# SamuelSchlesinger/anonymous-credit-tokens

Measured on NVIDIA B200. Metric: spend_verify_refund_per_sec, higher is better.
Workload: dtype u32 limbs (256-bit modular integer)

## Files before the change

### anonymous-credit-tokens_b200/csrc/act_device.cuh

```cuda
#pragma once
#include "blake3.cuh"
#include "fe25519.cuh"
#include "ge25519.cuh"
#include "sc25519.cuh"

#define ACT_ST_OK 0
#define ACT_ST_INVALID_ISSUANCE_REQUEST_PROOF 1
#define ACT_ST_INVALID_ISSUANCE_RESPONSE_PROOF 2
#define ACT_ST_INVALID_REFUND_PROOF 4
#define ACT_ST_IDENTITY_POINT 6
#define ACT_ST_INVALID_CLIENT_SPEND_PROOF 7
#define ACT_ST_DECODE_INVALID_POINT 0x81

#define ACT_FLAG_BAD_POINT 1u
#define ACT_FLAG_IDENTITY 2u
#define ACT_FLAG_BAD_PROOF 4u

#define ACT_L 128
#define ACT_PROOF_WORDS (526 * 8)
#define ACT_ITEMS 390
#define ACT_ITEM_WORDS (ACT_ITEMS * 8)
#define ACT_SPEND_BYTES 15784u
#define ACT_SPEND_CHUNKS 16

#ifndef ACT_FB_BITS
#define ACT_FB_BITS 13
#endif
#ifndef ACT_FB_BITS_HOT
#define ACT_FB_BITS_HOT 16
#endif
#define ACT_FB_PART 512
#define ACT_FB_BATCH 16
#if defined(__CUDACC__)
#define ACT_HD __host__ __device__ __forceinline__
#else
#define ACT_HD static inline
#endif
struct fb_tab {
    const ge_niels* p;
    u32 bits, win, ent;
};
ACT_HD u32 fb_win_of(u32 bits) { return (253u + bits) / bits; }
ACT_HD u32 fb_ent_of(u32 bits) { return (1u << (bits - 1)) + 1u; }
ACT_HD size_t fb_size_of(u32 bits) { return (size_t)fb_win_of(bits) * fb_ent_of(bits); }
ACT_HD u32 fb_parts_of(u32 bits) { u32 n = fb_ent_of(bits) - 1; return n >= ACT_FB_PART ? n / ACT_FB_PART : 1; }
#define ACT_CT_WIN 64
#define ACT_CT_ENT 9
#define ACT_CT_SIZE (ACT_CT_WIN * ACT_CT_ENT)

#ifndef ACT_RANGE_SPLIT
#define ACT_RANGE_SPLIT 4
#endif

#define ACT_BASE_G 0
#define ACT_BASE_H1 1
#define ACT_BASE_H2 2
#define ACT_BASE_H3 3
#define ACT_BASE_W 4
#define ACT_FB_BASES 5

struct act_ctx {
    fb_tab fb[ACT_FB_BASES];
    const ge_niels* ct_g;
    sc x;
    ge W;
    ge W_half;
    u32 h_enc[3][8];
    u32 prefix[4][48];
    u32 prefix_len[4];
};
#define ACT_TR_REQUEST 0
#define ACT_TR_RESPOND 1
#define ACT_TR_REFUND 2
#define ACT_TR_SPEND 3

#if ACT_PTX
#define ACT_ATOMIC_OR(p, v) atomicOr((p), (v))
#else
#define ACT_ATOMIC_OR(p, v) (*(p) |= (v))
#endif

ACT_FN void load8(u32* w, const u32* p) {
#if ACT_PTX
    uint4 a = __ldg(reinterpret_cast<const uint4*>(p));
    uint4 b = __ldg(reinterpret_cast<const uint4*>(p) + 1);
    w[0] = a.x; w[1] = a.y; w[2] = a.z; w[3] = a.w; w[4] = b.x; w[5] = b.y; w[6] = b.z; w[7] = b.w;
#else
    for (int i = 0; i < 8; i++) w[i] = p[i];
#endif
}
ACT_FN void store8(u32* p, const u32* w) {
#if ACT_PTX
    reinterpret_cast<uint4*>(p)[0] = make_uint4(w[0], w[1], w[2], w[3]);
    reinterpret_cast<uint4*>(p)[1] = make_uint4(w[4], w[5], w[6], w[7]);
#else
    for (int i = 0; i < 8; i++) p[i] = w[i];
#endif
}
ACT_FN void load8_rw(u32* w, const u32* p) {
#if ACT_PTX
    uint4 a = reinterpret_cast<const uint4*>(p)[0];
    uint4 b = reinterpret_cast<const uint4*>(p)[1];
    w[0] = a.x; w[1] = a.y; w[2] = a.z; w[3] = a.w; w[4] = b.x; w[5] = b.y; w[6] = b.z; w[7] = b.w;
#else
    for (int i = 0; i < 8; i++) w[i] = p[i];
#endif
}
ACT_FN void store8_zero(u32* p) {
    u32 z[8] = {0, 0, 0, 0, 0, 0, 0, 0};
    store8(p, z);
}
ACT_FN sc load_scalar(const u32* p) { u32 w[8]; load8(w, p); return sc_from_words(w); }
// ... 141 lines not shown
        if (k < M - 1) {
            ACT_NOUNROLL for (int d = 0; d < 4 * WIN; d++) Q = ge_dbl_u<VT>(Q, d == 4 * WIN - 1);
        }
    }
}
template <int M>
ACT_FN ge vb_mul_split_neg(const vb_table* t, const sc& s) {
    const int WIN = 64 / M;
    sc b = sc_bias<4>(s);
    ge a = ge_identity();
    ACT_NOUNROLL for (int i = WIN - 1; i >= 0; i--) {
        if (i != WIN - 1) {
            ACT_NOUNROLL for (int d = 0; d < 4; d++) {
#if ACT_PREFETCH >= 2
                if (d == 3) {
                    int d0 = sc_digit<4>(b, i);
                    prefetch_line(&t[0].e[d0 < 0 ? -d0 : d0]);
                }
#endif
                a = ge_dbl_u<true>(a, d == 3);
            }
        }
        ACT_NOUNROLL for (int k = 0; k < M; k++) {
            if (k + 1 < M) {
                int dn = sc_digit<4>(b, (k + 1) * WIN + i);
                prefetch_line(&t[k + 1].e[dn < 0 ? -dn : dn]);
            }
            int dk = sc_digit<4>(b, k * WIN + i);
            a = ge_add_cached_u<true>(a, tab_load(&t[k], (u32)(dk < 0 ? -dk : dk)), dk < 0 ? 0u : 1u, k + 1 < M || i == 0);
        }
    }
    return a;
}
#ifndef ACT_RANGE_BUCKETS
#define ACT_RANGE_BUCKETS 1
#endif
#if ACT_RANGE_BUCKETS
ACT_FN u32* bucket_ptr(vb_table* t, u32 idx) { return reinterpret_cast<u32*>(&t[idx / 9].e[idx % 9]); }
ACT_FN void bucket_store(vb_table* t, u32 idx, const ge& p) {
    u32* q = bucket_ptr(t, idx);
    store8(q, p.X.v); store8(q + 8, p.Y.v); store8(q + 16, p.Z.v); store8(q + 24, p.T.v);
}
ACT_FN ge bucket_load(vb_table* t, u32 idx) {
    ge p;
    const u32* q = bucket_ptr(t, idx);
    load8_rw(p.X.v, q); load8_rw(p.Y.v, q + 8); load8_rw(p.Z.v, q + 16); load8_rw(p.T.v, q + 24);
    return p;
}
#ifndef ACT_BUCKET_SKIP0
#define ACT_BUCKET_SKIP0 0
#endif
ACT_FN void vb_pair_buckets_fill(const ge& P, const sc& s0, const sc& s1, vb_table* t) {
    sc b0 = sc_bias<4>(s0), b1 = sc_bias<4>(s1);
    {
        ge id = ge_identity();
        ACT_NOUNROLL for (u32 k = 0; k < 18; k++) bucket_store(t, k, id);
    }
    ge Q = P;
    ACT_NOUNROLL for (int i = 0; i < 64; i++) {
        ge_cached Qc = ge_to_cached(Q);
        ACT_NOUNROLL for (int r = 0; r < 2; r++) {
            int d = sc_digit<4>(r ? b1 : b0, i);
#if ACT_BUCKET_SKIP0
            u32 ad = (u32)(d < 0 ? -d : d);
            u32 idx = 9u * (u32)r + (ad ? ad : 1u);
            if (i + 1 < 64 || r == 0) {
                int dn = r ? sc_digit<4>(b0, i + 1) : sc_digit<4>(b1, i);
                u32 an = (u32)(dn < 0 ? -dn : dn);
                prefetch_line(bucket_ptr(t, 9u * (u32)(r ^ 1) + (an ? an : 1u)));
            }
            ge B = bucket_load(t, idx);
            B = ge_add_cached_u<true>(B, Qc, d < 0 ? 0u : 1u, true);
            if (ad) bucket_store(t, idx, B);
#else
            u32 idx = 9u * (u32)r + (u32)(d < 0 ? -d : d);
            if (i + 1 < 64 || r == 0) {
                int dn = r ? sc_digit<4>(b0, i + 1) : sc_digit<4>(b1, i);
                prefetch_line(bucket_ptr(t, 9u * (u32)(r ^ 1) + (u32)(dn < 0 ? -dn : dn)));
            }
            ge B = bucket_load(t, idx);
            B = ge_add_cached_u<true>(B, Qc, d < 0 ? 0u : 1u, true);
            bucket_store(t, idx, B);
#endif
        }
        if (i + 1 < 64) {
            ACT_NOUNROLL for (int k = 0; k < 4; k++) Q = ge_dbl_u<true>(Q, k == 3);
        }
    }
}
ACT_FN ge vb_pair_buckets_sum(vb_table* t, int r) {
    ge S = bucket_load(t, 9u * (u32)r + 8u), R = S;
    ACT_NOUNROLL for (u32 d = 7; d >= 1; d--) {
        S = ge_add_cached_u<true>(S, ge_to_cached(bucket_load(t, 9u * (u32)r + d)), 0u, true);
        R = ge_add_cached_u<true>(R, ge_to_cached(S), 0u, true);
    }
    return R;
}
#endif

ACT_NOINLINE void vb_mul_ct_(ge* out, const ge* P, const sc* s) {
    vb_table t;
    vb_table_build(&t, *P);
    sc b = sc_bias<4>(*s);
    ge acc = ge_identity();
    ACT_NOUNROLL for (int i = 63; i >= 0; i--) {
        if (i != 63) {
            acc = ge_dbl(acc, false); acc = ge_dbl(acc, false); acc = ge_dbl(acc, false); acc = ge_dbl(acc, true);
        }
        acc = ge_add_cached(acc, vb_lookup_ct(&t, sc_digit<4>(b, i)));
    }
    *out = acc;
}

#ifndef ACT_SIGN_SPLIT
#define ACT_SIGN_SPLIT 4
#endif
ACT_NOINLINE void vb_mul2_ct_(ge* out1, ge* out2, const ge* P, const sc* s1, const sc* s2) {
    const int M = ACT_SIGN_SPLIT, WIN = 64 / M;
    vb_table t[M];
    vb_split_tables<M>(*P, t);
    ACT_NOUNROLL for (int w = 0; w < 2; w++) {
        sc b = sc_bias<4>(w ? *s2 : *s1);
        ge a = ge_identity();
        ACT_NOUNROLL for (int i = WIN - 1; i >= 0; i--) {
            if (i != WIN - 1) {
                ACT_NOUNROLL for (int d = 0; d < 4; d++) a = ge_dbl_u(a, d == 3);
            }
            ACT_NOUNROLL for (int k = 0; k < M; k++) a = ge_add_cached_u(a, vb_lookup_ct(&t[k], sc_digit<4>(b, k * WIN + i)), 0u, k + 1 < M || i == 0);
        }
        if (w) *out2 = a; else *out1 = a;
// ... 154 lines not shown
    vb_table_build(&t[1], *X_A);
    sc ss[2] = {*z, *gamma};
    bool ng[2] = {false, true};
    ge Y_A = vb_mul_multi<2>(t, ss, ng);
    ge Y_G = fb_accumulate(ge_identity(), C->fb[ACT_BASE_G], sc_sub(*z, sc_mul(*e, *gamma)), false);
    Y_G = fb_accumulate(Y_G, C->fb[ACT_BASE_W], *gamma, true);
    tr_small tr;
    u32 w[8];
    tr_init(&tr, C, kind);
    if (kind == ACT_TR_RESPOND) tr_add32(&tr, c->v);
    tr_add32(&tr, e->v);
    tr_add32(&tr, A_words);
    ristretto_encode_(w, X_A); tr_add32(&tr, w);
    ristretto_encode_(w, &X_G); tr_add32(&tr, w);
    ristretto_encode_(w, &Y_A); tr_add32(&tr, w);
    ristretto_encode_(w, &Y_G); tr_add32(&tr, w);
    sc g2 = tr_challenge(&tr);
    return sc_eq(g2, *gamma);
}
ACT_FN void issuance_check_thread(const act_ctx* C, size_t i, const u32* Kin, const u32* resp, u8* status) {
    const u32* rs = resp + 40 * i;
    ge K, A;
    u32 aw[8];
    load8(aw, rs);
    u32 valid = load_point(&K, Kin + 8 * i) & ristretto_decode_(&A, aw);
    sc e = load_scalar(rs + 8), gamma = load_scalar(rs + 16), z = load_scalar(rs + 24), c = load_scalar(rs + 32);
    ge X_A = ge_add(K, ge_basepoint());
    X_A = fb_accumulate(X_A, C->fb[ACT_BASE_H1], c, false);
    u32 ok = dleq_check_(C, ACT_TR_RESPOND, &c, &e, &gamma, &z, aw, &A, &X_A);
    status[i] = (u8)(!valid ? ACT_ST_DECODE_INVALID_POINT : (ok ? ACT_ST_OK : ACT_ST_INVALID_ISSUANCE_RESPONSE_PROOF));
}

ACT_FN void spend_range_thread(const act_ctx* C, size_t p, int j, const u32* proofs, u32* items, u32* com_niels, u32* flags,
                               vb_table* tabs , u32* cpts ) {
    const u32* pf = proofs + (size_t)ACT_PROOF_WORDS * p;
    u32* it = items + (size_t)ACT_ITEM_WORDS * p;
    u32 cw[8];
    load8(cw, pf + 8 * (4 + j));
    ge P;
    u32 valid = ristretto_decode_(&P, cw);
    if (!valid) ACT_ATOMIC_OR(&flags[p], ACT_FLAG_BAD_POINT);
    store8(it + 8 * (5 + j), cw);
    {
        ge_niels n = ge_affine_to_niels(P.X, P.Y);
        u32* cn = com_niels + ((size_t)ACT_L * p + j) * 24;
        store_fe(cn, n.ypx); store_fe(cn + 8, n.ymx); store_fe(cn + 16, n.xy2d);
    }
#if ACT_RANGE_BUCKETS
    {
        sc g0 = load_scalar(pf + 8 * (140 + j));
        sc g1 = sc_sub(load_scalar(pf + 8 * 132), g0);
        vb_pair_buckets_fill(P, sc_half(g0), sc_half(g1), tabs);
    }
#else
    vb_split_tables<ACT_RANGE_SPLIT, true>(P, tabs);
#endif
    u32* cp = cpts + ((size_t)2 * ACT_L * p + 2 * j) * 32;
    ACT_NOUNROLL for (int b = 0; b < 2; b++) {
#if ACT_RANGE_BUCKETS
        ge Q = vb_pair_buckets_sum(tabs, b);
#else
        sc gb = load_scalar(pf + 8 * (140 + j));
        if (b) gb = sc_sub(load_scalar(pf + 8 * 132), gb);
        gb = sc_half(gb);
        ge Q = vb_mul_split_neg<ACT_RANGE_SPLIT>(tabs, gb);
#endif
        ACT_NOUNROLL for (int t = 0; t < 2; t++) {
            int tab;
            sc s;
            if (t == 0) { tab = ACT_BASE_H3; s = load_scalar(pf + 8 * (268 + 2 * j + b)); }
            else { if (!b) continue; tab = ACT_BASE_H1; s = sc_sub(load_scalar(pf + 8 * 132), load_scalar(pf + 8 * (140 + j))); }
            Q = fb_accumulate(Q, C->fb[tab], sc_half(s), false);
        }
        store_fe(cp + 32 * b, Q.X); store_fe(cp + 32 * b + 8, Q.Y); store_fe(cp + 32 * b + 16, Q.Z); store_fe(cp + 32 * b + 24, Q.T);
    }
}

#ifndef ACT_ENC_BATCH
#define ACT_ENC_BATCH 64
#endif
ACT_FN void spend_encode_thread(const act_ctx* C, size_t p, int part, const u32* cpts, u32* items, int pts = 2 * ACT_L, int item0 = 133) {
    (void)C;
    const u32* src = cpts + ((size_t)pts * p + (size_t)part * ACT_ENC_BATCH) * 32;
    u32* dst = items + (size_t)ACT_ITEM_WORDS * p + 8 * (item0 + part * ACT_ENC_BATCH);
    fe prefix[ACT_ENC_BATCH];
    fe acc = fe_one();
    ACT_NOUNROLL for (int i = 0; i < ACT_ENC_BATCH; i++) {
        ge P;
        load_fe(&P.X, src + 32 * i); load_fe(&P.Y, src + 32 * i + 8); load_fe(&P.Z, src + 32 * i + 16); load_fe(&P.T, src + 32 * i + 24);
        ge_dbl_enc s = ge_dbl_enc_prepare(P);
        fe t = fe_mul(s.eg, s.fh);
        t = fe_select(t, fe_one(), fe_is_zero(t));
        prefix[i] = acc;
        acc = fe_mul(acc, t);
    }
    fe inv = fe_invert(acc);
    ACT_NOUNROLL for (int i = ACT_ENC_BATCH - 1; i >= 0; i--) {
        ge P;
        load_fe(&P.X, src + 32 * i); load_fe(&P.Y, src + 32 * i + 8); load_fe(&P.Z, src + 32 * i + 16); load_fe(&P.T, src + 32 * i + 24);
        ge_dbl_enc s = ge_dbl_enc_prepare(P);
        fe t = fe_mul(s.eg, s.fh);
        u32 zero = fe_is_zero(t);
        t = fe_select(t, fe_one(), zero);
        fe inv_i = fe_mul(inv, prefix[i]);
        inv = fe_mul(inv, t);
        u32 w[8];
        ge_dbl_enc_finish(w, s, inv_i);
        ACT_UNROLL for (int k = 0; k < 8; k++) w[k] = zero ? 0u : w[k];
// ... 233 lines not shown
```

### anonymous-credit-tokens_b200/csrc/act_engine.cu

```cuda
#include <cuda_runtime.h>
#include <stdio.h>
#include <stdlib.h>
#include <string.h>
#include <sys/random.h>

#include <mutex>
#include <string>
#include <thread>
#include <vector>

#include "../../include/act_engine.h"
#include "act_device.cuh"
#include "act_aux.cuh"
#include "act_prove.cuh"
#include "act_store.cuh"

#ifndef ACT_ISSUE_BLOCK
#define ACT_ISSUE_BLOCK 128
#endif
#ifndef ACT_HEAD_BLOCK
#define ACT_HEAD_BLOCK 64
#endif
#ifndef ACT_SIGN_BLOCK
#define ACT_SIGN_BLOCK 64
// ... 15 lines not shown
__global__ void __launch_bounds__(ACT_SIGN_BLOCK, ACT_SIGN_BPS) refund_sign_seq_kernel(const act_ctx* C, size_t n, const u32* proofs, const u32* rnd, const u32* kprime, const u8* status,
                                                                           u32* refunds, u32* nullifiers, const u32* rnd_index, const u32* kwords) {
    size_t p = (size_t)blockIdx.x * blockDim.x + threadIdx.x;
    if (p < n) refund_sign_thread(C, p, proofs, rnd, kprime, status, refunds, nullifiers, rnd_index, kwords);
}
__global__ void __launch_bounds__(ACT_ISSUE_BLOCK, ACT_ISSUE_BPS) issuance_check_kernel(const act_ctx* C, size_t n, const u32* K, const u32* resp, u8* status) {
    size_t i = (size_t)blockIdx.x * blockDim.x + threadIdx.x;
    if (i < n) issuance_check_thread(C, i, K, resp, status);
}
#ifndef ACT_RANGE_BLOCKS_PER_SM
#define ACT_RANGE_BLOCKS_PER_SM 4
#endif
#ifndef ACT_RANGE_DYNAMIC
#define ACT_RANGE_DYNAMIC 1
#endif
#ifndef ACT_RANGE_BLOCK
#define ACT_RANGE_BLOCK 128
#endif
#if !ACT_RANGE_DYNAMIC && ACT_RANGE_BLOCK != ACT_L
#error "the static work distribution needs one block per proof"
#endif
#define ACT_RANGE_UNITS (ACT_L / 32)
#if ACT_RANGE_TRACE
__device__ unsigned long long act_trace_buf[4096 * 4];
__device__ __forceinline__ unsigned long long act_gtime() { unsigned long long t; asm volatile("mov.u64 %0, %%globaltimer;" : "=l"(t)); return t; }
#endif
#ifdef ACT_RANGE_MAXREG
#define ACT_RANGE_BOUNDS __maxnreg__(ACT_RANGE_MAXREG)
#else
#define ACT_RANGE_BOUNDS __launch_bounds__(ACT_RANGE_BLOCK, ACT_RANGE_BLOCKS_PER_SM)
#endif
__global__ void ACT_RANGE_BOUNDS spend_range_kernel(const act_ctx* C, size_t m, const u32* proofs, u32* items, u32* com_niels, u32* flags, vb_table* tabs, u32* cpts, u32* counter) {
    vb_table* mine = tabs + ((size_t)blockIdx.x * ACT_RANGE_BLOCK + threadIdx.x) * ACT_RANGE_SPLIT;
#if ACT_RANGE_TRACE
    unsigned long long t0 = act_gtime(), units = 0;
#endif
#if ACT_RANGE_DYNAMIC
    const u32 lane = threadIdx.x & 31u, total = (u32)m * ACT_RANGE_UNITS;
    for (;;) {
        u32 unit = 0;
        if (lane == 0) unit = atomicAdd(counter, 1u);
        unit = __shfl_sync(0xffffffffu, unit, 0);
        if (unit >= total) break;
        spend_range_thread(C, unit / ACT_RANGE_UNITS, (int)((unit % ACT_RANGE_UNITS) * 32 + lane), proofs, items, com_niels, flags, mine, cpts);
#if ACT_RANGE_TRACE
        units++;
#endif
    }
#else
    (void)counter;
    for (size_t p = blockIdx.x; p < m; p += gridDim.x) {
        spend_range_thread(C, p, threadIdx.x, proofs, items, com_niels, flags, mine, cpts);
#if ACT_RANGE_TRACE
        units++;
#endif
    }
#endif
#if ACT_RANGE_TRACE
    if ((threadIdx.x & 31) == 0) {
        unsigned smid; asm volatile("mov.u32 %0, %%smid;" : "=r"(smid));
        unsigned w = blockIdx.x * (ACT_RANGE_BLOCK / 32) + threadIdx.x / 32;
        if (w < 4096) { act_trace_buf[4 * w] = smid; act_trace_buf[4 * w + 1] = t0; act_trace_buf[4 * w + 2] = act_gtime(); act_trace_buf[4 * w + 3] = units; }
    }
#endif
}
#if ACT_RANGE_TRACE
extern "C" __attribute__((visibility("default"))) int act_debug_read_trace(unsigned long long* out, size_t n) {
    return (int)cudaMemcpyFromSymbol(out, act_trace_buf, n * sizeof(unsigned long long));
}
#endif
#define ACT_ENC_BLOCK 128
#define ACT_ENC_PARTS (2 * ACT_L / ACT_ENC_BATCH)
__global__ void __launch_bounds__(ACT_ENC_BLOCK, 4) spend_encode_kernel(const act_ctx* C, size_t m, const u32* cpts, u32* items, int pts, int item0) {
    size_t t = (size_t)blockIdx.x * blockDim.x + threadIdx.x;
    int parts = pts / ACT_ENC_BATCH;
    if (t < m * parts) spend_encode_thread(C, t / parts, (int)(t % parts), cpts, items, pts, item0);
}
__global__ void __launch_bounds__(ACT_L, 4) prove_range_kernel(const act_ctx* C, prove_rng R, size_t m, const u32* tokens, const u32* charges, u32* cpts) {
    for (size_t p = blockIdx.x; p < m; p += gridDim.x) prove_range_thread(C, &R, p, p, threadIdx.x, tokens, charges, cpts);
}
__global__ void __launch_bounds__(ACT_HEAD_BLOCK, ACT_HEAD_BPS) prove_head_kernel(const act_ctx* C, prove_rng R, size_t m, const u32* tokens, u32* items, u32* aux, u8* status) {
    size_t p = (size_t)blockIdx.x * blockDim.x + threadIdx.x;
    if (p < m) prove_head_thread(C, &R, p, p, tokens, items, aux, status);
}
__global__ void __launch_bounds__(ACT_HASH_BLOCK) prove_challenge_kernel(size_t m, const u32* cvs, u32* gammas) {
// ... 1556 lines not shown
```

### anonymous-credit-tokens_b200/csrc/fe25519.cuh

```cuda
#pragma once
#include <stdint.h>

#if defined(__CUDACC__)
#define ACT_FN __device__ __forceinline__
#define ACT_NOINLINE __device__ __noinline__
#define ACT_CONST __device__ __constant__ const
#else
#define ACT_FN static inline
#define ACT_NOINLINE static
#define ACT_CONST static const
#endif

#if defined(__CUDA_ARCH__)
#define ACT_PTX 1
#define ACT_UNROLL _Pragma("unroll")
#define ACT_NOUNROLL _Pragma("unroll 1")
#else
#define ACT_PTX 0
#define ACT_UNROLL
#define ACT_NOUNROLL
#endif

#ifndef ACT_REDUCE_ALT
#define ACT_REDUCE_ALT 1
// ... 548 lines not shown
        "madc.lo.cc.u32 %14, %23, %23, %14;\n\t"
        "madc.hi.u32 %15, %23, %23, %15;"
        : "+r"(r[0]), "+r"(r[1]), "+r"(r[2]), "+r"(r[3]), "+r"(r[4]), "+r"(r[5]), "+r"(r[6]), "+r"(r[7]), "+r"(r[8]), "+r"(r[9]), "+r"(r[10]), "+r"(r[11]), "+r"(r[12]), "+r"(r[13]), "+r"(r[14]), "+r"(r[15])
        : "r"(a.v[0]), "r"(a.v[1]), "r"(a.v[2]), "r"(a.v[3]), "r"(a.v[4]), "r"(a.v[5]), "r"(a.v[6]), "r"(a.v[7]));
}

#endif

ACT_FN fe fe_sq_inl(const fe& a) {
#if ACT_PTX
    u32 r[16];
    fe_sq_wide(r, a);
    return fe_reduce512(r);
#else
    return fe_mul_inl(a, a);
#endif
}
#ifndef ACT_FE_CALLS
#define ACT_FE_CALLS 1
#endif
#if ACT_FE_CALLS
ACT_NOINLINE fe fe_mul(fe a, fe b) { return fe_mul_inl(a, b); }
ACT_NOINLINE fe fe_sq(fe a) { return fe_sq_inl(a); }
#else
ACT_FN fe fe_mul(const fe& a, const fe& b) { return fe_mul_inl(a, b); }
ACT_FN fe fe_sq(const fe& a) { return fe_sq_inl(a); }
#endif

ACT_FN fe fe_sqn(fe a, int n) {
    ACT_NOUNROLL for (int i = 0; i < n; i++) a = fe_sq(a);
    return a;
}

ACT_FN fe fe_canon(const fe& a) {
    fe r = a;
    u32 top = r.v[7] >> 31;
    r.v[7] &= 0x7fffffffu;
    u64 c = (u64)top * 19u;
    ACT_UNROLL for (int i = 0; i < 8; i++) { c += r.v[i]; r.v[i] = (u32)c; c >>= 32; }
    fe t;
    c = 19;
    ACT_UNROLL for (int i = 0; i < 8; i++) { c += r.v[i]; t.v[i] = (u32)c; c >>= 32; }
    u32 ge = t.v[7] >> 31;
    t.v[7] &= 0x7fffffffu;
    u32 m = 0u - ge;
    ACT_UNROLL for (int i = 0; i < 8; i++) r.v[i] = (r.v[i] & ~m) | (t.v[i] & m);
    return r;
}
ACT_FN u32 fe_is_negative(const fe& a) { return fe_canon(a).v[0] & 1u; }
ACT_FN u32 fe_is_zero(const fe& a) {
    fe c = fe_canon(a);
    u32 o = 0;
    ACT_UNROLL for (int i = 0; i < 8; i++) o |= c.v[i];
    return o == 0;
}
ACT_FN u32 fe_eq(const fe& a, const fe& b) { return fe_is_zero(fe_sub(a, b)); }
ACT_FN fe fe_select(const fe& x, const fe& y, u32 b) {
    fe r;
    u32 m = 0u - (b & 1u);
    ACT_UNROLL for (int i = 0; i < 8; i++) r.v[i] = (x.v[i] & ~m) | (y.v[i] & m);
    return r;
}
ACT_FN fe fe_cneg(const fe& x, u32 b) { return fe_select(x, fe_neg(x), b); }
ACT_FN fe fe_abs(const fe& x) { return fe_cneg(x, fe_is_negative(x)); }

ACT_FN fe fe_from_words(const u32* w) {
// ... 58 lines not shown
```

### anonymous-credit-tokens_b200/csrc/ge25519.cuh

```cuda
#pragma once
#include "fe25519.cuh"
#include "sc25519.cuh"

struct ge { fe X, Y, Z, T; };
struct ge_cached { fe YpX, YmX, Z, T2d; };
struct ge_niels { fe ypx, ymx, xy2d; };

ACT_FN ge ge_identity() { ge r; r.X = fe_zero(); r.Y = fe_one(); r.Z = fe_one(); r.T = fe_zero(); return r; }
ACT_FN ge ge_basepoint() { ge r; r.X = fe_const(FE_BX_); r.Y = fe_const(FE_BY_); r.Z = fe_one(); r.T = fe_const(FE_BT_); return r; }
ACT_FN ge_cached ge_cached_identity() { ge_cached r; r.YpX = fe_one(); r.YmX = fe_one(); r.Z = fe_one(); r.T2d = fe_zero(); return r; }
ACT_FN ge_niels ge_niels_identity() { ge_niels r; r.ypx = fe_one(); r.ymx = fe_one(); r.xy2d = fe_zero(); return r; }

ACT_FN ge_cached ge_to_cached(const ge& p) {
    ge_cached r;
    r.YpX = fe_add(p.Y, p.X); r.YmX = fe_sub(p.Y, p.X); r.Z = p.Z; r.T2d = fe_mul(p.T, FE_D2);
    return r;
}
ACT_FN ge ge_neg(const ge& p) { ge r; r.X = fe_neg(p.X); r.Y = p.Y; r.Z = p.Z; r.T = fe_neg(p.T); return r; }

#ifndef ACT_ALU_COPY
#define ACT_ALU_COPY 0
#endif
#if defined(__CUDACC__) && ACT_ALU_COPY
__device__ u32 act_zero_word = 0;
#endif
#if ACT_PTX && ACT_ALU_COPY
ACT_FN u32 act_zero() { return __ldg(&act_zero_word); }
ACT_FN fe fe_cp(const fe& a, u32 z) {
    fe r;
    ACT_UNROLL for (int i = 0; i < 8; i++) asm("xor.b32 %0, %1, %2;" : "=r"(r.v[i]) : "r"(a.v[i]), "r"(z));
    return r;
}
ACT_FN fe fe_mul_c(const fe& a, const fe& b, u32 z) {
    fe r = (ACT_ALU_COPY & 1) ? fe_mul(fe_cp(a, z), fe_cp(b, z)) : fe_mul(a, b);
    return (ACT_ALU_COPY & 2) ? fe_cp(r, z) : r;
}
ACT_FN fe fe_sq_c(const fe& a, u32 z) {
    fe r = (ACT_ALU_COPY & 1) ? fe_sq(fe_cp(a, z)) : fe_sq(a);
    return (ACT_ALU_COPY & 2) ? fe_cp(r, z) : r;
}
#else
ACT_FN u32 act_zero() { return 0; }
ACT_FN fe fe_mul_c(const fe& a, const fe& b, u32) { return fe_mul(a, b); }
ACT_FN fe fe_sq_c(const fe& a, u32) { return fe_sq(a); }
#endif

#ifndef ACT_GE_CALLS
#define ACT_GE_CALLS 0
#endif
#if ACT_GE_CALLS
#define ACT_GE_FN ACT_NOINLINE
// ... 57 lines not shown
    fe G0 = fe_add_x<VT>(ZZ2, TT), F0 = fe_sub_x<VT>(ZZ2, TT);
    fe G = fe_select(G0, F0, neg), F = fe_select(F0, G0, neg);
    ge r;
    r.X = GE_MUL(E, F); r.Y = GE_MUL(H, G); r.Z = GE_MUL(G, F); r.T = GE_MUL(E, H);
    return r;
}
ACT_FN ge ge_add(const ge& p, const ge& q) { return ge_add_cached(p, ge_to_cached(q)); }
ACT_FN ge ge_sub(const ge& p, const ge& q) { return ge_add_cached(p, ge_to_cached(ge_neg(q))); }

ACT_GE_FN ge ge_dbl_t(ge p) {
    u32 zc_ = act_zero(); (void)zc_;
    fe XX = GE_SQ(p.X), YY = GE_SQ(p.Y), ZZ = GE_SQ(p.Z);
    fe ZZ2 = fe_dbl_tt(ZZ);
    fe XpY2 = GE_SQ(fe_add(p.X, p.Y));
    fe Yc = fe_add_tt(YY, XX), Zc = fe_sub(YY, XX);
    fe Xc = fe_sub(XpY2, Yc), Tc = fe_sub(ZZ2, Zc);
    ge r;
    r.X = GE_MUL(Xc, Tc); r.Y = GE_MUL(Yc, Zc); r.Z = GE_MUL(Zc, Tc); r.T = GE_MUL(Xc, Yc);
    return r;
}
ACT_GE_FN ge ge_dbl_not(ge p) {
    u32 zc_ = act_zero(); (void)zc_;
    fe XX = GE_SQ(p.X), YY = GE_SQ(p.Y), ZZ = GE_SQ(p.Z);
    fe ZZ2 = fe_dbl_tt(ZZ);
    fe XpY2 = GE_SQ(fe_add(p.X, p.Y));
    fe Yc = fe_add_tt(YY, XX), Zc = fe_sub(YY, XX);
    fe Xc = fe_sub(XpY2, Yc), Tc = fe_sub(ZZ2, Zc);
    ge r;
    r.X = GE_MUL(Xc, Tc); r.Y = GE_MUL(Yc, Zc); r.Z = GE_MUL(Zc, Tc); r.T = p.T;
    return r;
}
ACT_FN ge ge_dbl(const ge& p, bool want_t) { return want_t ? ge_dbl_t(p) : ge_dbl_not(p); }

template <bool VT = false>
ACT_FN ge ge_dbl_u(const ge& p, bool want_t) {
    u32 zc_ = act_zero(); (void)zc_;
    fe XX = GE_SQ(p.X), YY = GE_SQ(p.Y);
    fe Yc = fe_add_tt(YY, XX), Zc = fe_sub_x<VT>(YY, XX);
    fe ZZ = GE_SQ(p.Z);
    fe ZZ2 = fe_dbl_tt(ZZ);
    fe Tc = fe_sub_x<VT>(ZZ2, Zc);
    fe XpY2 = GE_SQ(fe_add_x<VT>(p.X, p.Y));
    fe Xc = fe_sub_x<VT>(XpY2, Yc);
    ge r;
    r.Y = GE_MUL(Yc, Zc); r.Z = GE_MUL(Tc, Zc); r.X = GE_MUL(Tc, Xc);
    r.T = p.T;
    if (want_t) r.T = GE_MUL(Xc, Yc);
    return r;
}

ACT_FN ge_cached ge_cached_cneg(const ge_cached& q, u32 neg) {
    ge_cached r;
    r.YpX = fe_select(q.YpX, q.YmX, neg); r.YmX = fe_select(q.YmX, q.YpX, neg);
    r.Z = q.Z; r.T2d = fe_select(q.T2d, fe_neg(q.T2d), neg);
    return r;
}
ACT_FN ge_niels ge_niels_cneg(const ge_niels& q, u32 neg) {
    ge_niels r;
    r.ypx = fe_select(q.ypx, q.ymx, neg); r.ymx = fe_select(q.ymx, q.ypx, neg);
    r.xy2d = fe_select(q.xy2d, fe_neg(q.xy2d), neg);
    return r;
}
ACT_FN ge_niels ge_affine_to_niels(const fe& x, const fe& y) {
    ge_niels r;
    r.ypx = fe_add(y, x); r.ymx = fe_sub(y, x); r.xy2d = fe_mul(fe_mul(x, y), FE_D2);
    return r;
}
ACT_FN ge_niels ge_to_niels(const ge& p) {
    fe zi = fe_invert(p.Z);
    return ge_affine_to_niels(fe_mul(p.X, zi), fe_mul(p.Y, zi));
}
ACT_FN ge ge_from_niels(const ge_niels& n) {
    ge r;
    r.Y = fe_add(n.ypx, n.ymx); r.X = fe_sub(n.ypx, n.ymx); r.Z = fe_add(fe_one(), fe_one());
    fe zi = fe_invert(r.Z);
    fe x = fe_mul(r.X, zi), y = fe_mul(r.Y, zi);
    r.X = x; r.Y = y; r.Z = fe_one(); r.T = fe_mul(x, y);
    return r;
// ... 93 lines not shown
```

Before: 205,900.

## Share proof-wide wNAF scalar across warp in range bucket multiplication

Each range thread previously ran bucket-method multiplications for two per-thread scalars, g0 and (total − g0), with 18 buckets. Now one lane per warp computes a width-5 wNAF of the shared total scalar into shared memory. Every thread accumulates its own g0 buckets plus sparse wNAF buckets along one doubling chain, and the second output is derived as total·P − g0·P from the first sum. This cuts per-thread point additions, since wNAF digits are sparse, but it adds warp syncs, divergent loop control (doubling every bit with branches) and a serial wNAF computation on lane 0.

```diff
diff --git a/anonymous-credit-tokens_b200/csrc/act_device.cuh b/anonymous-credit-tokens_b200/csrc/act_device.cuh
--- a/anonymous-credit-tokens_b200/csrc/act_device.cuh
+++ b/anonymous-credit-tokens_b200/csrc/act_device.cuh
@@ -76,8 +76,10 @@
 
 #if ACT_PTX
 #define ACT_ATOMIC_OR(p, v) atomicOr((p), (v))
+#define ACT_SYNCWARP() __syncwarp()
 #else
 #define ACT_ATOMIC_OR(p, v) (*(p) |= (v))
+#define ACT_SYNCWARP() ((void)0)
 #endif
 
 ACT_FN void load8(u32* w, const u32* p) {
@@ -288,6 +290,7 @@
 #ifndef ACT_RANGE_BUCKETS
 #define ACT_RANGE_BUCKETS 1
 #endif
+#define ACT_NAF_LEN 256
 #if ACT_RANGE_BUCKETS
 ACT_FN u32* bucket_ptr(vb_table* t, u32 idx) { return reinterpret_cast<u32*>(&t[idx / 9].e[idx % 9]); }
 ACT_FN void bucket_store(vb_table* t, u32 idx, const ge& p) {
@@ -300,54 +303,68 @@
     load8_rw(p.X.v, q); load8_rw(p.Y.v, q + 8); load8_rw(p.Z.v, q + 16); load8_rw(p.T.v, q + 24);
     return p;
 }
-#ifndef ACT_BUCKET_SKIP0
-#define ACT_BUCKET_SKIP0 0
-#endif
-ACT_FN void vb_pair_buckets_fill(const ge& P, const sc& s0, const sc& s1, vb_table* t) {
-    sc b0 = sc_bias<4>(s0), b1 = sc_bias<4>(s1);
+#define ACT_NAF_W 5
+#define ACT_NAF_BUCKETS (1 << (ACT_NAF_W - 2))
+ACT_FN void sc_wnaf(signed char* naf, const sc& s) {
+    u32 carry = 0;
+    int i = 0;
+    ACT_NOUNROLL while (i < 253) {
+        u32 w = (u32)i >> 5, sh = (u32)i & 31u;
+        if (((s.v[w] >> sh) & 1u) == carry) { naf[i++] = 0; continue; }
+        u32 hi = (w + 1 < 8) ? s.v[w + 1] : 0u;
+        u32 raw = (sh ? ((s.v[w] >> sh) | (hi << (32u - sh))) : s.v[w]) & ((1u << ACT_NAF_W) - 1u);
+        int v = (int)(raw + carry);
+        carry = v > (1 << (ACT_NAF_W - 1)) ? 1u : 0u;
+        naf[i] = (signed char)(v - (int)(carry << ACT_NAF_W));
+        ACT_NOUNROLL for (int m = 1; m < ACT_NAF_W && i + m < 253; m++) naf[i + m] = 0;
+        i += ACT_NAF_W;
+    }
+}
+ACT_FN void vb_pair_buckets_fill(const ge& P, const sc& s0, const signed char* naf, vb_table* t) {
+    sc b0 = sc_bias<4>(s0);
     {
         ge id = ge_identity();
-        ACT_NOUNROLL for (u32 k = 0; k < 18; k++) bucket_store(t, k, id);
+        ACT_NOUNROLL for (u32 k = 0; k < 9 + ACT_NAF_BUCKETS; k++) bucket_store(t, k, id);
     }
     ge Q = P;
-    ACT_NOUNROLL for (int i = 0; i < 64; i++) {
+    ACT_NOUNROLL for (int k = 0; k < 253; k++) {
+        const bool r0 = (k & 3) == 0;
+        const int n = naf[k];
+        const int d = r0 ? sc_digit<4>(b0, k >> 2) : 0;
+        if (r0) prefetch_line(bucket_ptr(t, (u32)(d < 0 ? -d : d)));
+        if (n) prefetch_line(bucket_ptr(t, 9u + (u32)((n < 0 ? -n : n) >> 1)));
+        if (k) Q = ge_dbl_u<true>(Q, r0 || n);
+        if (!r0 && !n) continue;
         ge_cached Qc = ge_to_cached(Q);
-        ACT_NOUNROLL for (int r = 0; r < 2; r++) {
-            int d = sc_digit<4>(r ? b1 : b0, i);
-#if ACT_BUCKET_SKIP0
-            u32 ad = (u32)(d < 0 ? -d : d);
-            u32 idx = 9u * (u32)r + (ad ? ad : 1u);
-            if (i + 1 < 64 || r == 0) {
-                int dn = r ? sc_digit<4>(b0, i + 1) : sc_digit<4>(b1, i);
-                u32 an = (u32)(dn < 0 ? -dn : dn);
-                prefetch_line(bucket_ptr(t, 9u * (u32)(r ^ 1) + (an ? an : 1u)));
-            }
+        ACT_NOUNROLL for (int r = r0 ? 0 : 1; r < (n ? 2 : 1); r++) {
+            u32 idx, neg;
+            if (r == 0) { idx = (u32)(d < 0 ? -d : d); neg = d < 0 ? 0u : 1u; }
+            else { idx = 9u + (u32)((n < 0 ? -n : n) >> 1); neg = n < 0 ? 1u : 0u; }
             ge B = bucket_load(t, idx);
-            B = ge_add_cached_u<true>(B, Qc, d < 0 ? 0u : 1u, true);
-            if (ad) bucket_store(t, idx, B);
-#else
-            u32 idx = 9u * (u32)r + (u32)(d < 0 ? -d : d);
-            if (i + 1 < 64 || r == 0) {
-                int dn = r ? sc_digit<4>(b0, i + 1) : sc_digit<4>(b1, i);
-                prefetch_line(bucket_ptr(t, 9u * (u32)(r ^ 1) + (u32)(dn < 0 ? -dn : dn)));
-            }
-            ge B = bucket_load(t, idx);
-            B = ge_add_cached_u<true>(B, Qc, d < 0 ? 0u : 1u, true);
+            B = ge_add_cached_u<true>(B, Qc, neg, true);
             bucket_store(t, idx, B);
-#endif
-        }
-        if (i + 1 < 64) {
-            ACT_NOUNROLL for (int k = 0; k < 4; k++) Q = ge_dbl_u<true>(Q, k == 3);
-        }
-    }
-}
-ACT_FN ge vb_pair_buckets_sum(vb_table* t, int r) {
-    ge S = bucket_load(t, 9u * (u32)r + 8u), R = S;
+        }
+    }
+}
+ACT_FN ge vb_pair_buckets_sum(vb_table* t) {
+    ge S = bucket_load(t, 8u), R = S;
     ACT_NOUNROLL for (u32 d = 7; d >= 1; d--) {
-        S = ge_add_cached_u<true>(S, ge_to_cached(bucket_load(t, 9u * (u32)r + d)), 0u, true);
+        S = ge_add_cached_u<true>(S, ge_to_cached(bucket_load(t, d)), 0u, true);
         R = ge_add_cached_u<true>(R, ge_to_cached(S), 0u, true);
     }
     return R;
+}
+ACT_FN ge vb_pair_shared_second(vb_table* t, const ge& R0) {
+    ge S = bucket_load(t, 9u + ACT_NAF_BUCKETS - 1), R = S;
+    ACT_NOUNROLL for (u32 e = ACT_NAF_BUCKETS - 2; e >= 1; e--) {
+        S = ge_add_cached_u<true>(S, ge_to_cached(bucket_load(t, 9u + e)), 0u, true);
+        R = ge_add_cached_u<true>(R, ge_to_cached(S), 0u, true);
+    }
+    S = ge_add_cached_u<true>(S, ge_to_cached(bucket_load(t, 9u)), 0u, true);
+    S = ge_add_cached_u<true>(S, ge_to_cached(R0), 0u, true);
+    R = ge_dbl_u<true>(R, true);
+    R = ge_add_cached_u<true>(R, ge_to_cached(S), 0u, true);
+    return ge_neg(R);
 }
 #endif
 
@@ -569,7 +586,8 @@
 }
 
 ACT_FN void spend_range_thread(const act_ctx* C, size_t p, int j, const u32* proofs, u32* items, u32* com_niels, u32* flags,
-                               vb_table* tabs , u32* cpts ) {
+                               vb_table* tabs , u32* cpts ,
+                               signed char* naf, bool naf_writer) {
     const u32* pf = proofs + (size_t)ACT_PROOF_WORDS * p;
     u32* it = items + (size_t)ACT_ITEM_WORDS * p;
     u32 cw[8];
@@ -584,18 +602,24 @@
         store_fe(cn, n.ypx); store_fe(cn + 8, n.ymx); store_fe(cn + 16, n.xy2d);
     }
 #if ACT_RANGE_BUCKETS
-    {
-        sc g0 = load_scalar(pf + 8 * (140 + j));
-        sc g1 = sc_sub(load_scalar(pf + 8 * 132), g0);
-        vb_pair_buckets_fill(P, sc_half(g0), sc_half(g1), tabs);
-    }
+    ACT_SYNCWARP();
+    if (naf_writer) sc_wnaf(naf, sc_half(load_scalar(pf + 8 * 132)));
+    ACT_SYNCWARP();
+    vb_pair_buckets_fill(P, sc_half(load_scalar(pf + 8 * (140 + j))), naf, tabs);
 #else
+    (void)naf; (void)naf_writer;
     vb_split_tables<ACT_RANGE_SPLIT, true>(P, tabs);
 #endif
     u32* cp = cpts + ((size_t)2 * ACT_L * p + 2 * j) * 32;
     ACT_NOUNROLL for (int b = 0; b < 2; b++) {
 #if ACT_RANGE_BUCKETS
-        ge Q = vb_pair_buckets_sum(tabs, b);
+        ge Q;
+        if (b == 0) {
+            Q = vb_pair_buckets_sum(tabs);
+            bucket_store(tabs, 0, Q);
+        } else {
+            Q = vb_pair_shared_second(tabs, bucket_load(tabs, 0));
+        }
 #else
         sc gb = load_scalar(pf + 8 * (140 + j));
         if (b) gb = sc_sub(load_scalar(pf + 8 * 132), gb);
@@ -611,6 +635,11 @@
         }
         store_fe(cp + 32 * b, Q.X); store_fe(cp + 32 * b + 8, Q.Y); store_fe(cp + 32 * b + 16, Q.Z); store_fe(cp + 32 * b + 24, Q.T);
     }
+}
+ACT_FN void spend_range_thread(const act_ctx* C, size_t p, int j, const u32* proofs, u32* items, u32* com_niels, u32* flags,
+                               vb_table* tabs, u32* cpts) {
+    signed char naf[ACT_NAF_LEN];
+    spend_range_thread(C, p, j, proofs, items, com_niels, flags, tabs, cpts, naf, true);
 }
 
 #ifndef ACT_ENC_BATCH
diff --git a/anonymous-credit-tokens_b200/csrc/act_engine.cu b/anonymous-credit-tokens_b200/csrc/act_engine.cu
--- a/anonymous-credit-tokens_b200/csrc/act_engine.cu
+++ b/anonymous-credit-tokens_b200/csrc/act_engine.cu
@@ -71,6 +71,9 @@
 #endif
 __global__ void ACT_RANGE_BOUNDS spend_range_kernel(const act_ctx* C, size_t m, const u32* proofs, u32* items, u32* com_niels, u32* flags, vb_table* tabs, u32* cpts, u32* counter) {
     vb_table* mine = tabs + ((size_t)blockIdx.x * ACT_RANGE_BLOCK + threadIdx.x) * ACT_RANGE_SPLIT;
+    __shared__ signed char naf[ACT_RANGE_BLOCK / 32][ACT_NAF_LEN];
+    signed char* my_naf = naf[threadIdx.x >> 5];
+    const bool naf_writer = (threadIdx.x & 31u) == 0;
 #if ACT_RANGE_TRACE
     unsigned long long t0 = act_gtime(), units = 0;
 #endif
@@ -81,7 +84,7 @@
         if (lane == 0) unit = atomicAdd(counter, 1u);
         unit = __shfl_sync(0xffffffffu, unit, 0);
         if (unit >= total) break;
-        spend_range_thread(C, unit / ACT_RANGE_UNITS, (int)((unit % ACT_RANGE_UNITS) * 32 + lane), proofs, items, com_niels, flags, mine, cpts);
+        spend_range_thread(C, unit / ACT_RANGE_UNITS, (int)((unit % ACT_RANGE_UNITS) * 32 + lane), proofs, items, com_niels, flags, mine, cpts, my_naf, naf_writer);
 #if ACT_RANGE_TRACE
         units++;
 #endif
@@ -89,7 +92,7 @@
 #else
     (void)counter;
     for (size_t p = blockIdx.x; p < m; p += gridDim.x) {
-        spend_range_thread(C, p, threadIdx.x, proofs, items, com_niels, flags, mine, cpts);
+        spend_range_thread(C, p, threadIdx.x, proofs, items, com_niels, flags, mine, cpts, my_naf, naf_writer);
 #if ACT_RANGE_TRACE
         units++;
 #endif
```

Measured after the change: 206,800, median of 6. Within noise of the previous version (+0.5%).

## Share range-proof challenge scalar via NAF buckets instead of per-bit subtraction

Applied to the files above, without the earlier changes.

Range-proof commitment scalar multiplication now uses the bit challenge g0 and the shared challenge c separately, instead of g0 and c−g0. The second multiple is rebuilt as c·P − g0·P, with c·P accumulated through a sparse width-5 NAF digit stream during the same doubling chain. The goal is fewer bucket additions than a dense signed-4-bit second scalar. The cost is more complex control flow, extra bucket storage for the NAF digits, and a final combination step in the bucket sum.

```diff
diff --git a/anonymous-credit-tokens_b200/csrc/act_device.cuh b/anonymous-credit-tokens_b200/csrc/act_device.cuh
--- a/anonymous-credit-tokens_b200/csrc/act_device.cuh
+++ b/anonymous-credit-tokens_b200/csrc/act_device.cuh
@@ -349,6 +349,96 @@
     }
     return R;
 }
+
+#ifndef ACT_RANGE_SHARED_CHALLENGE
+#define ACT_RANGE_SHARED_CHALLENGE 1
+#endif
+#if ACT_RANGE_SHARED_CHALLENGE
+#if ACT_BUCKET_SKIP0
+#error "ACT_BUCKET_SKIP0 applies to the two-scalar bucket form only (ACT_RANGE_SHARED_CHALLENGE=0)"
+#endif
+#define ACT_NAF_NONE 256
+ACT_FN void naf5_next(const u32* s, int* k, int* d, u32* carry) {
+    int i = *k;
+    for (;;) {
+        if (i >= 256) { *k = ACT_NAF_NONE; return; }
+        u32 w = (s[i >> 5] ^ (0u - *carry)) >> (i & 31);
+        if (w) {
+#if ACT_PTX
+            i += __ffs((int)w) - 1;
+#else
+            i += __builtin_ctz(w);
+#endif
+            break;
+        }
+        i = (i | 31) + 1;
+    }
+    u32 lo = s[i >> 5] >> (i & 31);
+    if ((i & 31) > 27 && i < 224) lo |= s[(i >> 5) + 1] << (32 - (i & 31));
+    int win = (int)(lo & 31u) + (int)*carry;
+    *carry = (win & 16) ? 1u : 0u;
+    *d = win - (int)(*carry << 5);
+    *k = i;
+}
+ACT_FN void vb_pair_shared_fill(const ge& P, const sc& s0, const sc& sg, vb_table* t) {
+    {
+        ge id = ge_identity();
+        ACT_NOUNROLL for (u32 k = 0; k < 18; k++) if (k != 9) bucket_store(t, k, id);
+    }
+    sc b0 = sc_bias<4>(s0);
+    u32* sgw = bucket_ptr(t, 9);
+    store8(sgw, sg.v);
+    int nk = 0, nd = 0;
+    u32 carry = 0;
+    naf5_next(sgw, &nk, &nd, &carry);
+    {
+        int d = sc_digit<4>(b0, 0);
+        prefetch_line(bucket_ptr(t, (u32)(d < 0 ? -d : d)));
+    }
+    ge Q = P;
+    int k = 0;
+    ACT_NOUNROLL for (;;) {
+        bool win = (k & 3) == 0, naf = k == nk;
+        ge_cached Qc = ge_to_cached(Q);
+        ACT_NOUNROLL for (int r = 0; r < 2; r++) {
+            if (r ? !naf : !win) continue;
+            int d = r ? nd : sc_digit<4>(b0, k >> 2);
+            u32 ad = (u32)(d < 0 ? -d : d);
+            u32 idx = r ? 9u + ((ad + 1) >> 1) : ad;
+            if (!r && k < 252) {
+                int dn = sc_digit<4>(b0, (k >> 2) + 1);
+                prefetch_line(bucket_ptr(t, (u32)(dn < 0 ? -dn : dn)));
+            }
+            ge B = bucket_load(t, idx);
+            B = ge_add_cached_u<true>(B, Qc, d < 0 ? 0u : 1u, true);
+            bucket_store(t, idx, B);
+        }
+        if (naf) {
+            nk += 5;
+            naf5_next(sgw, &nk, &nd, &carry);
+            if (nk != ACT_NAF_NONE) prefetch_line(bucket_ptr(t, 9u + (((u32)(nd < 0 ? -nd : nd) + 1) >> 1)));
+        }
+        int e = (k | 3) + 1;
+        if (nk < e) e = nk;
+        if (e > 253) break;
+        ACT_NOUNROLL for (; k < e; k++) Q = ge_dbl_u<true>(Q, k + 1 == e);
+    }
+}
+ACT_FN ge vb_pair_shared_sum(vb_table* t, int r) {
+    ge S = bucket_load(t, 9u * (u32)r + 8u), R = S;
+    ACT_NOUNROLL for (u32 d = 7; d >= 1; d--) {
+        S = ge_add_cached_u<true>(S, ge_to_cached(bucket_load(t, 9u * (u32)r + d)), 0u, true);
+        R = ge_add_cached_u<true>(R, ge_to_cached(S), 0u, true);
+    }
+    if (r == 0) {
+        bucket_store(t, 9, R);
+        return R;
+    }
+    R = ge_dbl_u<true>(R, true);
+    R = ge_add_cached_u<true>(R, ge_to_cached(S), 1u, true);
+    return ge_add_cached_u<true>(R, ge_to_cached(bucket_load(t, 9)), 1u, true);
+}
+#endif
 #endif
 
 ACT_NOINLINE void vb_mul_ct_(ge* out, const ge* P, const sc* s) {
@@ -583,7 +673,9 @@
         u32* cn = com_niels + ((size_t)ACT_L * p + j) * 24;
         store_fe(cn, n.ypx); store_fe(cn + 8, n.ymx); store_fe(cn + 16, n.xy2d);
     }
-#if ACT_RANGE_BUCKETS
+#if ACT_RANGE_BUCKETS && ACT_RANGE_SHARED_CHALLENGE
+    vb_pair_shared_fill(P, sc_half(load_scalar(pf + 8 * (140 + j))), sc_half(load_scalar(pf + 8 * 132)), tabs);
+#elif ACT_RANGE_BUCKETS
     {
         sc g0 = load_scalar(pf + 8 * (140 + j));
         sc g1 = sc_sub(load_scalar(pf + 8 * 132), g0);
@@ -594,7 +686,9 @@
 #endif
     u32* cp = cpts + ((size_t)2 * ACT_L * p + 2 * j) * 32;
     ACT_NOUNROLL for (int b = 0; b < 2; b++) {
-#if ACT_RANGE_BUCKETS
+#if ACT_RANGE_BUCKETS && ACT_RANGE_SHARED_CHALLENGE
+        ge Q = vb_pair_shared_sum(tabs, b);
+#elif ACT_RANGE_BUCKETS
         ge Q = vb_pair_buckets_sum(tabs, b);
 #else
         sc gb = load_scalar(pf + 8 * (140 + j));
```

Measured after the change: 205,800 before, 209,700 after, median of 6. +1.9%, better.

## Precompute cached chain points and use small-constant cached conversion in bucket MSM

Applied to the files above, without the earlier changes.

The bucket fill now computes all 64 doubled chain points first and stores them in cached form in the thread's scratch, instead of interleaving doubling with the bucket adds. The cached conversion replaces the full field multiply by 2d with small-constant multiplies on a scaled, negated representation (the lambda trick), and the sign flags are flipped to match. The doubling in the precompute uses inlined field ops, and the range split grows to 10 tables so the scratch can hold the 64 extra points. This trades a larger per-thread local-memory footprint and more stores and loads for fewer full multiplies and a better-separated dependency chain.

```diff
diff --git a/anonymous-credit-tokens_b200/csrc/act_device.cuh b/anonymous-credit-tokens_b200/csrc/act_device.cuh
--- a/anonymous-credit-tokens_b200/csrc/act_device.cuh
+++ b/anonymous-credit-tokens_b200/csrc/act_device.cuh
@@ -48,8 +48,11 @@
 #define ACT_CT_ENT 9
 #define ACT_CT_SIZE (ACT_CT_WIN * ACT_CT_ENT)
 
+#ifndef ACT_RANGE_BUCKETS
+#define ACT_RANGE_BUCKETS 1
+#endif
 #ifndef ACT_RANGE_SPLIT
-#define ACT_RANGE_SPLIT 4
+#define ACT_RANGE_SPLIT (ACT_RANGE_BUCKETS ? 10 : 4)
 #endif
 
 #define ACT_BASE_G 0
@@ -285,10 +288,8 @@
     }
     return a;
 }
-#ifndef ACT_RANGE_BUCKETS
-#define ACT_RANGE_BUCKETS 1
-#endif
 #if ACT_RANGE_BUCKETS
+static_assert(ACT_RANGE_SPLIT * 9 >= 18 + 64, "the bucket form keeps 18 buckets and 64 chain points in the thread's scratch");
 ACT_FN u32* bucket_ptr(vb_table* t, u32 idx) { return reinterpret_cast<u32*>(&t[idx / 9].e[idx % 9]); }
 ACT_FN void bucket_store(vb_table* t, u32 idx, const ge& p) {
     u32* q = bucket_ptr(t, idx);
@@ -300,52 +301,51 @@
     load8_rw(p.X.v, q); load8_rw(p.Y.v, q + 8); load8_rw(p.Z.v, q + 16); load8_rw(p.T.v, q + 24);
     return p;
 }
-#ifndef ACT_BUCKET_SKIP0
-#define ACT_BUCKET_SKIP0 0
-#endif
+ACT_FN void cached_store(vb_table* t, u32 idx, const ge_cached& c) {
+    u32* q = bucket_ptr(t, idx);
+    store8(q, c.YpX.v); store8(q + 8, c.YmX.v); store8(q + 16, c.Z.v); store8(q + 24, c.T2d.v);
+}
+ACT_FN ge_cached cached_load(vb_table* t, u32 idx) {
+    ge_cached c;
+    const u32* q = bucket_ptr(t, idx);
+    load8_rw(c.YpX.v, q); load8_rw(c.YmX.v, q + 8); load8_rw(c.Z.v, q + 16); load8_rw(c.T2d.v, q + 24);
+    return c;
+}
 ACT_FN void vb_pair_buckets_fill(const ge& P, const sc& s0, const sc& s1, vb_table* t) {
+    {
+        ge Q = P;
+        ACT_NOUNROLL for (u32 i = 0;; i++) {
+            cached_store(t, 18u + i, ge_to_cached_neg_pub(Q));
+            if (i == 63) break;
+            ACT_NOUNROLL for (int k = 0; k < 4; k++) Q = ge_dbl_u<true, true>(Q, k == 3);
+        }
+    }
     sc b0 = sc_bias<4>(s0), b1 = sc_bias<4>(s1);
     {
         ge id = ge_identity();
         ACT_NOUNROLL for (u32 k = 0; k < 18; k++) bucket_store(t, k, id);
     }
-    ge Q = P;
     ACT_NOUNROLL for (int i = 0; i < 64; i++) {
-        ge_cached Qc = ge_to_cached(Q);
+        ge_cached Qc = cached_load(t, 18u + (u32)i);
+        if (i + 1 < 64) prefetch_line(bucket_ptr(t, 19u + (u32)i));
         ACT_NOUNROLL for (int r = 0; r < 2; r++) {
             int d = sc_digit<4>(r ? b1 : b0, i);
-#if ACT_BUCKET_SKIP0
-            u32 ad = (u32)(d < 0 ? -d : d);
-            u32 idx = 9u * (u32)r + (ad ? ad : 1u);
-            if (i + 1 < 64 || r == 0) {
-                int dn = r ? sc_digit<4>(b0, i + 1) : sc_digit<4>(b1, i);
-                u32 an = (u32)(dn < 0 ? -dn : dn);
-                prefetch_line(bucket_ptr(t, 9u * (u32)(r ^ 1) + (an ? an : 1u)));
-            }
-            ge B = bucket_load(t, idx);
-            B = ge_add_cached_u<true>(B, Qc, d < 0 ? 0u : 1u, true);
-            if (ad) bucket_store(t, idx, B);
-#else
             u32 idx = 9u * (u32)r + (u32)(d < 0 ? -d : d);
             if (i + 1 < 64 || r == 0) {
                 int dn = r ? sc_digit<4>(b0, i + 1) : sc_digit<4>(b1, i);
                 prefetch_line(bucket_ptr(t, 9u * (u32)(r ^ 1) + (u32)(dn < 0 ? -dn : dn)));
             }
             ge B = bucket_load(t, idx);
-            B = ge_add_cached_u<true>(B, Qc, d < 0 ? 0u : 1u, true);
+            B = ge_add_cached_u<true>(B, Qc, d < 0 ? 1u : 0u, true);
             bucket_store(t, idx, B);
-#endif
-        }
-        if (i + 1 < 64) {
-            ACT_NOUNROLL for (int k = 0; k < 4; k++) Q = ge_dbl_u<true>(Q, k == 3);
         }
     }
 }
 ACT_FN ge vb_pair_buckets_sum(vb_table* t, int r) {
     ge S = bucket_load(t, 9u * (u32)r + 8u), R = S;
     ACT_NOUNROLL for (u32 d = 7; d >= 1; d--) {
-        S = ge_add_cached_u<true>(S, ge_to_cached(bucket_load(t, 9u * (u32)r + d)), 0u, true);
-        R = ge_add_cached_u<true>(R, ge_to_cached(S), 0u, true);
+        S = ge_add_cached_u<true>(S, ge_to_cached_neg_pub(bucket_load(t, 9u * (u32)r + d)), 1u, true);
+        R = ge_add_cached_u<true>(R, ge_to_cached_neg_pub(S), 1u, true);
     }
     return R;
 }
diff --git a/anonymous-credit-tokens_b200/csrc/fe25519.cuh b/anonymous-credit-tokens_b200/csrc/fe25519.cuh
--- a/anonymous-credit-tokens_b200/csrc/fe25519.cuh
+++ b/anonymous-credit-tokens_b200/csrc/fe25519.cuh
@@ -604,6 +604,31 @@
     return a;
 }
 
+ACT_FN fe fe_mul_small(const fe& a, u32 c) {
+    u32 t[9];
+#if ACT_PTX
+    u64 e0 = (u64)a.v[0] * c, e1 = (u64)a.v[2] * c, e2 = (u64)a.v[4] * c, e3 = (u64)a.v[6] * c;
+    u64 q0 = (u64)a.v[1] * c, q1 = (u64)a.v[3] * c, q2 = (u64)a.v[5] * c, q3 = (u64)a.v[7] * c;
+    t[0] = (u32)e0; t[1] = (u32)(e0 >> 32); t[2] = (u32)e1; t[3] = (u32)(e1 >> 32);
+    t[4] = (u32)e2; t[5] = (u32)(e2 >> 32); t[6] = (u32)e3; t[7] = (u32)(e3 >> 32); t[8] = 0;
+    asm("add.cc.u32 %0, %0, %8;\n\t"
+        "addc.cc.u32 %1, %1, %9;\n\t"
+        "addc.cc.u32 %2, %2, %10;\n\t"
+        "addc.cc.u32 %3, %3, %11;\n\t"
+        "addc.cc.u32 %4, %4, %12;\n\t"
+        "addc.cc.u32 %5, %5, %13;\n\t"
+        "addc.cc.u32 %6, %6, %14;\n\t"
+        "addc.u32 %7, %7, %15;"
+        : "+r"(t[1]), "+r"(t[2]), "+r"(t[3]), "+r"(t[4]), "+r"(t[5]), "+r"(t[6]), "+r"(t[7]), "+r"(t[8])
+        : "r"((u32)q0), "r"((u32)(q0 >> 32)), "r"((u32)q1), "r"((u32)(q1 >> 32)), "r"((u32)q2), "r"((u32)(q2 >> 32)), "r"((u32)q3), "r"((u32)(q3 >> 32)));
+#else
+    u64 k = 0;
+    for (int i = 0; i < 8; i++) { k += (u64)a.v[i] * c; t[i] = (u32)k; k >>= 32; }
+    t[8] = (u32)k;
+#endif
+    return fe_fold9(t);
+}
+
 ACT_FN fe fe_canon(const fe& a) {
     fe r = a;
     u32 top = r.v[7] >> 31;
diff --git a/anonymous-credit-tokens_b200/csrc/ge25519.cuh b/anonymous-credit-tokens_b200/csrc/ge25519.cuh
--- a/anonymous-credit-tokens_b200/csrc/ge25519.cuh
+++ b/anonymous-credit-tokens_b200/csrc/ge25519.cuh
@@ -17,6 +17,14 @@
     return r;
 }
 ACT_FN ge ge_neg(const ge& p) { ge r; r.X = fe_neg(p.X); r.Y = p.Y; r.Z = p.Z; r.T = fe_neg(p.T); return r; }
+#define GE_CACHED_LAMBDA 60833u
+#define GE_CACHED_LAMBDA_2D_NEG 121665u
+ACT_FN ge_cached ge_to_cached_neg_pub(const ge& p) {
+    ge_cached r;
+    r.YpX = fe_mul_small(fe_sub_v(p.Y, p.X), GE_CACHED_LAMBDA); r.YmX = fe_mul_small(fe_add_v(p.Y, p.X), GE_CACHED_LAMBDA);
+    r.Z = fe_mul_small(p.Z, GE_CACHED_LAMBDA); r.T2d = fe_mul_small(p.T, GE_CACHED_LAMBDA_2D_NEG);
+    return r;
+}
 
 #ifndef ACT_ALU_COPY
 #define ACT_ALU_COPY 0
@@ -140,18 +148,20 @@
 }
 ACT_FN ge ge_dbl(const ge& p, bool want_t) { return want_t ? ge_dbl_t(p) : ge_dbl_not(p); }
 
-template <bool VT = false>
+template <bool INL> ACT_FN fe ge_dbl_sq_(const fe& a, u32 zc_) { (void)zc_; return INL ? fe_sq_inl(a) : GE_SQ(a); }
+template <bool INL> ACT_FN fe ge_dbl_mul_(const fe& a, const fe& b, u32 zc_) { (void)zc_; return INL ? fe_mul_inl(a, b) : GE_MUL(a, b); }
+template <bool VT = false, bool INL = false>
 ACT_FN ge ge_dbl_u(const ge& p, bool want_t) {
     u32 zc_ = act_zero(); (void)zc_;
-    fe XX = GE_SQ(p.X), YY = GE_SQ(p.Y);
+    fe XX = ge_dbl_sq_<INL>(p.X, zc_), YY = ge_dbl_sq_<INL>(p.Y, zc_);
     fe Yc = fe_add_tt(YY, XX), Zc = fe_sub_x<VT>(YY, XX);
-    fe ZZ = GE_SQ(p.Z);
+    fe ZZ = ge_dbl_sq_<INL>(p.Z, zc_);
     fe ZZ2 = fe_dbl_tt(ZZ);
     fe Tc = fe_sub_x<VT>(ZZ2, Zc);
-    fe XpY2 = GE_SQ(fe_add_x<VT>(p.X, p.Y));
+    fe XpY2 = ge_dbl_sq_<INL>(fe_add_x<VT>(p.X, p.Y), zc_);
     fe Xc = fe_sub_x<VT>(XpY2, Yc);
     ge r;
-    r.Y = GE_MUL(Yc, Zc); r.Z = GE_MUL(Tc, Zc); r.X = GE_MUL(Tc, Xc);
+    r.Y = ge_dbl_mul_<INL>(Yc, Zc, zc_); r.Z = ge_dbl_mul_<INL>(Tc, Zc, zc_); r.X = ge_dbl_mul_<INL>(Tc, Xc, zc_);
     r.T = p.T;
     if (want_t) r.T = GE_MUL(Xc, Yc);
     return r;
```

New measurement: 206,000 before, 209,800 after (median of 6 runs). 1.02x the previous value.
